# Nexenta/edge-fuse

Measured on NVIDIA H100. Metric: GiB/s hash+LZ4+dedup on 64 KiB chunks, higher is better.
Workload: dtype u8

## Files before the change

edge_fuse_b200/csrc/kernels.cu:

```cuda
#include "kernels.h"
#include "common.cuh"
#include "fingerprint.cuh"
#include "lz4_encode.cuh"
#include "lz4_encode_ring.cuh"
#include <type_traits>
#include "lz4_decode.cuh"
#include "lz4_decode_cta.cuh"
#include "streamgen.cuh"

namespace cmb {


__host__ __device__ __forceinline__ unsigned long long fnv_addr(unsigned long long u, unsigned long long l) {
	unsigned long long h = 14695981039346656037ULL;
#pragma unroll
	for (int i = 0; i < 8; i++) { h = (h ^ ((u >> (8 * i)) & 0xFF)) * 0x100000001b3ULL; }
#pragma unroll
	for (int i = 0; i < 8; i++) { h = (h ^ ((l >> (8 * i)) & 0xFF)) * 0x100000001b3ULL; }
	return h;
}

__device__ __forceinline__ uint64_t home_slot(unsigned long long key, uint64_t cap) {
	unsigned long long z = key;
	z = (z ^ (z >> 32)) * 0xD6E8FEB86659FD93ULL;
// ... 282 lines not shown
constexpr float COST_FULL = 160.0f;
#ifdef CMB_ENC_TIMELINE
__device__ unsigned long long *g_enc_timeline;
__device__ __forceinline__ unsigned long long enc_clock() {
	unsigned long long t;
	asm volatile("mov.u64 %0, %%globaltimer;" : "=l"(t));
	return t;
}
#endif
__global__ void __launch_bounds__(COST_WARPS * 32, 4) k_cost(EncodeJob job) {
	__shared__ __align__(16) uint32_t smp[COST_WARPS][256 + 4];
	__shared__ uint16_t tab[COST_WARPS][COST_TAB];
	const int lane = threadIdx.x & 31, warp = threadIdx.x >> 5;
	uint32_t *s = smp[warp];
	uint16_t *h = tab[warp];
	const uint8_t *sb = reinterpret_cast<const uint8_t *>(s);
	const uint32_t o0 = ((uint32_t)lane & 3u) * 32u;
	const uint32_t win_stride = (job.nbytes / 8u) & ~15u;
	for (uint32_t i = blockIdx.x * COST_WARPS + warp; i < job.n; i += gridDim.x * COST_WARPS) {
		const uint4 *src = reinterpret_cast<const uint4 *>(job.pages + (size_t)i * job.page_stride + (lane >> 2) * win_stride + o0);
		const uint4 a = __ldg(src), c = __ldg(src + 1);
		bool live = true;
		if (job.slot_idx) {
			const uint32_t idx = job.slot_idx[i];
			live = idx != 0xffffffffu && job.table.slots[idx].seq == job.seq0 + job.seq_stride * i;
		}
		uint32_t bucket = 0;
		[[maybe_unused]] uint32_t est = 0;
		if (live) {
			const uint32_t w[9] = {a.x, a.y, a.z, a.w, c.x, c.y, c.z, c.w, __shfl_down_sync(CMB_FULL, a.x, 1)};
			__syncwarp();
			reinterpret_cast<uint4 *>(s)[2 * lane] = a;
			reinterpret_cast<uint4 *>(s)[2 * lane + 1] = c;
#pragma unroll
			for (uint32_t k = 0; k < 32; k++) {
				if (o0 + k >= COST_POS) break;
				const uint32_t g = __funnelshift_r(w[k >> 2], w[(k >> 2) + 1], (k & 3u) * 8u);
				h[(g * 2654435761u) >> 21] = (uint16_t)((uint32_t)lane * 32u + k);
			}
			__syncwarp();
			uint32_t starts = 0, lits = 0;
#pragma unroll
			for (uint32_t k = 0; k < 32; k++) {
				if (o0 + k >= COST_POS) break;
				const uint32_t p = (uint32_t)lane * 32u + k;
				const uint32_t g = __funnelshift_r(w[k >> 2], w[(k >> 2) + 1], (k & 3u) * 8u);
				const uint32_t q = h[(g * 2654435761u) >> 21] & 1023u;
				const bool m = q != p && (q & 127u) < COST_POS && __funnelshift_r(s[q >> 2], s[(q >> 2) + 1], (q & 3u) * 8u) == g;
				const bool cont = m && o0 + k > 0u && (q & 127u) > 0u && sb[p - 1] == sb[q - 1];
				starts += m && !cont;
				lits += !m;
			}
#pragma unroll
			for (int d = 16; d > 0; d >>= 1) {
				starts += __shfl_xor_sync(CMB_FULL, starts, d);
				lits += __shfl_xor_sync(CMB_FULL, lits, d);
			}
			const float cost = (float)starts + COST_LIT * (float)lits / (float)job.accel;
			bucket = min(ENC_BUCKETS - 1u, (uint32_t)(cost * ((float)ENC_BUCKETS / COST_FULL)));
			est = starts << 16 | lits;
		}
		if (lane == 0) {
			const uint32_t pos = atomicAdd(&job.work[1 + bucket], 1u);
			job.order[(size_t)bucket * job.n + pos] = i;
#ifdef CMB_ENC_TIMELINE
			if (g_enc_timeline) g_enc_timeline[4 * (size_t)i + 3] = (unsigned long long)bucket << 32 | est;
#endif
		}
	}
}

__device__ __noinline__ uint32_t enc_ticket_chunk(const unsigned int *work, const uint32_t *order, uint32_t n, uint32_t t, int lane) {
	uint32_t cum = lane < (int)ENC_BUCKETS ? work[ENC_BUCKETS - lane] : 0u;
#pragma unroll
	for (int d = 1; d < (int)ENC_BUCKETS; d <<= 1) {
		const uint32_t v = __shfl_up_sync(CMB_FULL, cum, d);
		if (lane >= d) cum += v;
	}
	const int k = __ffs(__ballot_sync(CMB_FULL, lane < (int)ENC_BUCKETS && t < cum)) - 1;
	const uint32_t before = __shfl_sync(CMB_FULL, cum, (k + 31) & 31);
	return order[(size_t)(ENC_BUCKETS - 1 - k) * n + (t - (k ? before : 0u))];
}

constexpr int ENC_PLAIN_WARPS = 7, ENC_PLAIN_CTAS = 2, ENC_RING_WARPS = 13;
template <bool WIDE, int ENC>
__global__ void __launch_bounds__(ENC == 1 ? ENC_RING_WARPS * 32 : ENC_PLAIN_WARPS * 32, ENC == 1 ? 1 : ENC_PLAIN_CTAS) k_encode(EncodeJob job) {
	extern __shared__ __align__(128) uint8_t smem[];
	const int lane = threadIdx.x & 31, warp = threadIdx.x >> 5;
	const uint32_t nwarps = blockDim.x >> 5;
	uint8_t *wsm = smem + (size_t)warp * LZ4_TABLE_BYTES;
	PageRing ring;
	if (ENC == 1)
		ring_setup(ring, smem + (size_t)nwarps * LZ4_TABLE_BYTES + (size_t)warp * RING_ALLOC,
		    smem + (size_t)nwarps * (LZ4_TABLE_BYTES + RING_ALLOC) + (size_t)warp * RING_MBAR_BYTES, lane);
	const uint32_t gw = blockIdx.x * (blockDim.x >> 5) + warp;
	const bool direct = job.slot_idx != nullptr && job.arena.seg_bytes != 0u && job.accel != 0u && gw < ARENA_SEG_SLOTS;
	const uint32_t worst = (uint32_t)((24u + job.stage_stride + 15u) & ~15ull);
	unsigned long long seg_cur = 0, seg_end = 0;
	if (direct && lane == 0) { seg_cur = job.arena.seg[2 * gw]; seg_end = job.arena.seg[2 * gw + 1]; }
#ifdef CMB_ENC_TIMELINE
	uint32_t prev = ~0u;
#endif
	for (;;) {
		uint32_t i = 0;
		if (lane == 0) i = atomicAdd(job.work, 1u);
		i = __shfl_sync(CMB_FULL, i, 0);
		if (i < job.n && job.order) i = enc_ticket_chunk(job.work, job.order, job.n, i, lane);
#ifdef CMB_ENC_TIMELINE
		if (lane == 0 && g_enc_timeline) {
			const unsigned long long t = enc_clock();
			if (prev != ~0u) g_enc_timeline[4 * (size_t)prev + 2] = t;
			if (i < job.n) { g_enc_timeline[4 * (size_t)i] = gw; g_enc_timeline[4 * (size_t)i + 1] = t; }
			prev = i;
		}
#endif
		if (i >= job.n) break;
		const bool store = job.slot_idx != nullptr;
		uint32_t idx = 0;
		if (store) {
			idx = job.slot_idx[i];
			bool live = idx != 0xffffffffu && job.table.slots[idx].seq == job.seq0 + job.seq_stride * i;
			if (!live) { if (lane == 0) job.lens[i] = -1; continue; }
		}
		const uint8_t *src = job.pages + (size_t)i * job.page_stride;
		uint64_t fp_hi = 0, fp_lo = 0;
		if (job.accel == 0) {
			if (job.fps) {
				warp_fingerprint128(src, job.nbytes, lane, fp_hi, fp_lo);
				if (lane == 0) { job.fps[2 * (size_t)i] = fp_hi; job.fps[2 * (size_t)i + 1] = fp_lo; }
			}
			if (lane == 0) job.lens[i] = 0;
			if (store) commit_record(job, i, idx, src, job.nbytes, 0, true, fp_hi, fp_lo, lane);
			continue;
		}
		uint8_t *dst = job.stage + (size_t)(store ? gw : i) * job.stage_stride;
		unsigned long long base = 0;
		int in_arena = 0;
		if (direct) {
			if (lane == 0) {
				if (seg_cur + worst > seg_end) {
					if (seg_end > seg_cur) atomicAdd(job.arena.garbage, seg_end - seg_cur);
					const unsigned long long off = atomicAdd(job.arena.head, (unsigned long long)job.arena.seg_bytes);
					if (off + job.arena.seg_bytes <= job.arena.size) { seg_cur = off; seg_end = off + job.arena.seg_bytes; }
					else { seg_cur = seg_end = 0; }
				}
				in_arena = seg_cur + worst <= seg_end;
				base = seg_cur;
			}
			in_arena = __shfl_sync(CMB_FULL, in_arena, 0);
			base = __shfl_sync(CMB_FULL, base, 0);
			if (in_arena) dst = job.arena.base + base + 24;
		}
		uint32_t clen, ck = 0xffffffffu;
		if (job.fps) {
			clen = lz4_encode_lean<WIDE, true, ENC == 1>(src, job.nbytes, dst, job.accel, wsm, ring, lane, fp_hi, fp_lo, ck);
			if (lane == 0) { job.fps[2 * (size_t)i] = fp_hi; job.fps[2 * (size_t)i + 1] = fp_lo; }
		} else {
			clen = lz4_encode_lean<WIDE, false, ENC == 1>(src, job.nbytes, dst, job.accel, wsm, ring, lane, fp_hi, fp_lo, ck);
		}
		if (lane == 0) job.lens[i] = (int32_t)clen;
		if (store) {
			__syncwarp();
			if (in_arena) {
				const uint32_t used = commit_direct(job, i, idx, base, clen, fp_hi, fp_lo, lane);
				if (lane == 0) seg_cur += used;
				ckpt_store(job, idx, base, clen, ck, lane);
			} else {
				const unsigned long long at = commit_record(job, i, idx, dst, clen, (int32_t)clen, false, fp_hi, fp_lo, lane);
				if (at != ~0ull) ckpt_store(job, idx, at, clen, ck, lane);
			}
		}
	}
	if (direct && lane == 0) { job.arena.seg[2 * gw] = seg_cur; job.arena.seg[2 * gw + 1] = seg_end; }
}

static int g_sm_count = 0;
int sm_count() {
	if (!g_sm_count) {
		int dev = 0;
		cudaGetDevice(&dev);
		cudaDeviceGetAttribute(&g_sm_count, cudaDevAttrMultiProcessorCount, dev);
		if (g_sm_count <= 0) g_sm_count = 132;
	}
	return g_sm_count;
}

static int launch_encode_kernel(const EncodeJob &job, bool ring, cudaStream_t st) {
	const bool wide = job.nbytes >= LZ4_NARROW_LIMIT;
	void (*const kern)(EncodeJob) = ring ? (wide ? k_encode<true, 1> : k_encode<false, 1>)
	                                     : (wide ? k_encode<true, 0> : k_encode<false, 0>);
	const int warps = ring ? ENC_RING_WARPS : ENC_PLAIN_WARPS, ctas_per_sm = ring ? 1 : ENC_PLAIN_CTAS;
	const size_t smem = (size_t)warps * (ring ? RING_WARP_SMEM : LZ4_TABLE_BYTES);
	CMB_CHECK(cudaFuncSetAttribute(kern, cudaFuncAttributeMaxDynamicSharedMemorySize, (int)smem));
	uint32_t grid = (uint32_t)(sm_count() * ctas_per_sm);
	uint32_t need = (job.n + warps - 1) / warps;
	if (grid > need) grid = need;
	kern<<<grid, warps * 32, smem, st>>>(job);
	CMB_CHECK(cudaGetLastError());
	return 0;
}

int launch_encode(const EncodeJob &job_in, cudaStream_t st) {
	if (job_in.n == 0) return 0;
	EncodeJob job = job_in;
	const bool ring = job.accel >= 1 && job.accel <= RING_MAX_ACCEL && job.nbytes < (1u << 24);
	const uint32_t resident = (uint32_t)sm_count() * (ring ? ENC_RING_WARPS : ENC_PLAIN_CTAS * ENC_PLAIN_WARPS);
	if (job.n <= resident || job.accel == 0 || job.nbytes < 1024u) job.order = nullptr;
	CMB_CHECK(cudaMemsetAsync(job.work, 0, (job.order ? 1 + ENC_BUCKETS : 1) * sizeof(unsigned int), st));
	if (job.order) {
		k_cost<<<(job.n + COST_WARPS - 1) / COST_WARPS, COST_WARPS * 32, 0, st>>>(job);
		CMB_CHECK(cudaGetLastError());
	}
	if (launch_encode_kernel(job, ring, st) != 0) return -1;
	return job.order ? 2 : 1;
}

#ifdef CMB_ENC_TIMELINE
extern "C" int cmb200_enc_timeline(void *buf) {
	return cudaMemcpyToSymbol(g_enc_timeline, &buf, sizeof(buf)) == cudaSuccess ? 0 : -1;
}
#endif


__global__ void __launch_bounds__(256, 8) k_decode(DecodeJob job) {
	const int lane = threadIdx.x & 31;
	const uint32_t i = blockIdx.x * (blockDim.x >> 5) + (threadIdx.x >> 5);
	if (i >= job.n) return;
	uint8_t *out = job.pages + (size_t)i * job.nbytes;
	if (job.rec_off) {
		if (job.status[i] != ST_HIT) return;
		const unsigned long long off = job.rec_off[i];
		const uint8_t *rec = (off & REC_HOST) ? job.host + (off & ~REC_HOST) : job.arena + off;
		if ((off & REC_HOST) && lane == 0) {
			atomicAdd(job.host_hits, 1ull);
			hot_log(job.hot, job.addr[2 * (size_t)i], job.addr[2 * (size_t)i + 1]);
		}
		uint32_t clen = job.vlen[i] - 1u;
		if (clen == 0) {
			warp_copy_ro(out, rec + 24, job.nbytes, lane);
			return;
		}
		int used = lz4_decode_warp(rec + 24, clen, out, job.nbytes, lane);
		if (used != (int)clen && lane == 0) job.status[i] = ST_BAD_DECODE;
	} else {
		int used = lz4_decode_warp(job.blocks + (size_t)i * job.block_stride, (uint32_t)job.lens[i], out,
		    job.nbytes, lane);
		if (lane == 0) job.status[i] = used;
	}
}

int launch_decode(const DecodeJob &job, cudaStream_t st) {
	if (job.n == 0) return 0;
	const int warps = 8;
	k_decode<<<(job.n + warps - 1) / warps, warps * 32, 0, st>>>(job);
	CMB_CHECK(cudaGetLastError());
	return 0;
}


constexpr uint32_t GS_THREADS = DC_THREADS;
constexpr uint32_t GS_CTRL = 128 + 1152;
static_assert(sizeof(DecodeCta) <= 1152, "decoder state fits its slot");
constexpr uint32_t GS_MAX_PAGE = 65536;
constexpr uint32_t GS_PAIR_MAX_PAGE = 131072;
struct GetShared {
	unsigned long long bar;
	unsigned long long off;
	int32_t st;
	uint32_t clen;
	uint32_t owner;
	uint32_t idx;
	uint32_t region;
	uint32_t sections;
	uint32_t ck[CKPT_WORDS];
};
static_assert(sizeof(GetShared) <= 128, "control block");
__host__ __device__ inline uint32_t gs_recbuf(uint32_t nbytes) { return (24u + nbytes + 1024u + 31u) & ~15u; }
bool get_small_supports(uint32_t nbytes) { return nbytes >= 64u && nbytes <= GS_PAIR_MAX_PAGE && (nbytes & 15u) == 0; }
size_t get_small_smem(uint32_t nbytes) {
	return nbytes > GS_MAX_PAGE ? GS_CTRL + gs_recbuf(nbytes) : GS_CTRL + gs_recbuf(nbytes) + nbytes;
}
uint32_t get_small_region_entries(uint32_t nbytes) { return dc_region(nbytes); }

__device__ __forceinline__ unsigned long long ldv64(const unsigned long long *p) { return *reinterpret_cast<const volatile unsigned long long *>(p); }
__device__ __forceinline__ uint32_t ldv32(const uint32_t *p) { return *reinterpret_cast<const volatile uint32_t *>(p); }

__device__ void gs_lookup(const GetJob &job, unsigned long long u, unsigned long long l, GetShared *sh) {
	int32_t st = ST_MISS;
	uint32_t clen = 0, owner = 0;
	unsigned long long off = 0;
	const uint32_t idx = table_find(job.table, fnv_addr(u, l));
	if (idx != 0xffffffffu) {
		const Slot *s = &job.table.slots[idx];
		const uint32_t vlen = ldv32(&s->vlen);
		const unsigned long long au = ldv64(&s->addr_u), al = ldv64(&s->addr_l);
		if (vlen != 0u) {
			if (au == u && al == l) { st = ST_HIT; __threadfence(); off = ldv64(&s->rec_off); clen = vlen - 1u; }
			else st = ST_BAD_ENTRY;
		} else {
			const unsigned long long ow = ldv64(&s->owner);
			if (ow != 0ull && au == u && al == l) {
				st = ST_REMOTE; owner = (uint32_t)ow;
				__threadfence();
				off = ldv64(&s->rec_off);
				const uint32_t len1 = ldv32(&s->alloc);
				clen = len1 ? len1 - 1u : 0xffffffffu;
			}
		}
	}
	sh->st = st; sh->clen = clen; sh->off = off; sh->owner = owner; sh->idx = idx;
}

__device__ uint32_t gs_region_take(const GetJob &job) {
	uint32_t smid;
	asm volatile("mov.u32 %0, %%smid;" : "=r"(smid));
	const uint32_t words = (job.pool_n + 31u) / 32u;
	for (uint32_t probe = 0; probe < (1u << 22); probe++) {
		const uint32_t w = (smid + probe) % words;
		const uint32_t live = w + 1u == words && (job.pool_n & 31u) ? (1u << (job.pool_n & 31u)) - 1u : 0xffffffffu;
		const uint32_t vacant = ~ldv32(&job.pool_bits[w]) & live;
		if (!vacant) continue;
		const uint32_t b = (uint32_t)__ffs(vacant) - 1u;
		if (!((atomicOr(&job.pool_bits[w], 1u << b) >> b) & 1u)) return w * 32u + b;
	}
	return 0xffffffffu;
}
__device__ void gs_region_give(const GetJob &job, uint32_t r) { atomicAnd(&job.pool_bits[r / 32u], ~(1u << (r & 31u))); }

__device__ void gs_sections(const GetJob &job, GetShared *sh, DecodeCta *dc, uint32_t clen, bool local) {
	const uint32_t n = job.nbytes, S = n / DC_CHAINS;
	bool use = false;
	if (local && job.table.ckpt) {
		const uint32_t *ck = job.table.ckpt + (size_t)sh->idx * CKPT_WORDS;
		const uint32_t want = ckpt_tag(sh->off, clen);
		if (ldv32(ck) == want) {
			__threadfence();
			for (uint32_t k = 1; k < CKPT_WORDS; k++) sh->ck[k] = ldv32(ck + k);
			__threadfence();
			use = ldv32(ck) == want;
		}
	}
	for (uint32_t c = 0; c < DC_CHAINS; c++) { dc->ip0[c] = 0xffffffffu; dc->op0[c] = 0; dc->op_end[c] = 0; dc->cnt[c] = 0; dc->ip1[c] = 0; dc->op1[c] = 0; }
	dc->err = 0;
	dc->ip0[0] = 0; dc->op0[0] = 0;
	uint32_t prev = 0;
	if (use) {
		for (uint32_t k = 1; k < DC_CHAINS; k++) {
			const uint32_t v = sh->ck[k];
			if (v == 0xffffffffu) continue;
			const uint32_t ip = v >> CKPT_POS_BITS, op = k * S + (v & ((1u << CKPT_POS_BITS) - 1u));
			if (ip >= clen || op >= n || op >= (k + 1u) * S || ip <= dc->ip0[prev]) { use = false; break; }
			dc->ip0[k] = ip; dc->op0[k] = op;
			dc->op_end[prev] = op;
			prev = k;
		}
	}
	if (!use) {
		for (uint32_t c = 1; c < DC_CHAINS; c++) dc->ip0[c] = 0xffffffffu;
		prev = 0;
	}
	dc->op_end[prev] = n;
	sh->sections = use ? DC_CHAINS : 1u;
}

__device__ bool gs_sections_fit(const DecodeCta *dc, uint32_t clen, uint32_t n) {
	if (dc->err) return false;
	uint32_t prev = 0;
	for (uint32_t c = 1; c < DC_CHAINS; c++) {
		if (dc->ip0[c] == 0xffffffffu) continue;
		if (dc->ip1[prev] != dc->ip0[c] || dc->op1[prev] != dc->op0[c]) return false;
		prev = c;
	}
// ... 819 lines not shown
```

edge_fuse_b200/csrc/lz4_encode.cuh:

```cuda
#pragma once
#include "common.cuh"
#include "fingerprint.cuh"

namespace cmb {

constexpr uint32_t LZ4_MIN_MATCH = 4;
constexpr uint32_t LZ4_TAIL_LITERALS = 5;
constexpr uint32_t LZ4_MATCH_FIND_MARGIN = 12;
constexpr uint32_t LZ4_MIN_INPUT = 13;
constexpr uint32_t LZ4_NARROW_LIMIT = 65536 + 11;
constexpr uint32_t LZ4_FAR = 65535;
constexpr uint32_t LZ4_TABLE_BYTES = 16384;

__device__ __forceinline__ uint32_t lz4_hash4(uint32_t v) { return (v * 2654435761u) >> 19; }
__device__ __forceinline__ uint32_t lz4_hash5(uint64_t v) {
	return (uint32_t)(((v << 24) * 889523592379ULL) >> 52);
}

__device__ __forceinline__ uint32_t lz4_probe_off(uint32_t k, uint32_t accel) {
	if (k == 0) return 0;
	uint32_t m = k - 1, q = m >> 6, r = m & 63u;
	return 1u + accel * m + 32u * q * (q - 1u) + q * r;
}

template <bool WIDE> struct Lz4Table;
template <> struct Lz4Table<false> {
	uint16_t *t;
	__device__ __forceinline__ uint32_t get(uint32_t h) const { return t[h]; }
	__device__ __forceinline__ void put(uint32_t h, uint32_t pos) const { t[h] = (uint16_t)pos; }
};
template <> struct Lz4Table<true> {
	uint32_t *t;
	__device__ __forceinline__ uint32_t get(uint32_t h) const { return t[h]; }
	__device__ __forceinline__ void put(uint32_t h, uint32_t pos) const { t[h] = pos; }
};

struct Lz4Around { uint32_t before, at, next; };
struct Lz4Words { uint32_t w0, w1, w2, w3, sh; };
__device__ __forceinline__ Lz4Words lz4_around_load(const uint8_t *src, uint32_t p) {
	const uint32_t a = p & ~3u;
	const uint32_t *q = reinterpret_cast<const uint32_t *>(src + a);
	Lz4Words w;
	w.w0 = __ldg(q - (a != 0u));
	w.w1 = __ldg(q); w.w2 = __ldg(q + 1); w.w3 = __ldg(q + 2);
	w.sh = (p & 3u) * 8u;
	return w;
}
__device__ __forceinline__ Lz4Around lz4_around_align(const Lz4Words &w) {
	Lz4Around r;
	r.before = __funnelshift_r(w.w0, w.w1, w.sh);
	r.at = __funnelshift_r(w.w1, w.w2, w.sh);
	r.next = __funnelshift_r(w.w2, w.w3, w.sh);
	return r;
}
__device__ __forceinline__ Lz4Around lz4_around(const uint8_t *src, uint32_t p) {
	return lz4_around_align(lz4_around_load(src, p));
}


__device__ __noinline__ uint32_t lz4_emit_len(uint8_t *dst, uint32_t op, uint32_t count, int lane) {
	uint32_t nff = count / 255u;
	for (uint32_t i = lane; i < nff; i += 32) dst[op + i] = 0xFF;
	if (lane == 0) dst[op + nff] = (uint8_t)(count - nff * 255u);
	return op + nff + 1;
}
__device__ __forceinline__ uint32_t lz4_len_bytes(uint32_t count) { return count >= 15u ? (count - 15u) / 255u + 1u : 0u; }
__device__ __forceinline__ uint32_t lz4_seq_bytes(uint32_t lit, uint32_t mc) {
	return 3u + lit + lz4_len_bytes(lit) + lz4_len_bytes(mc);
}

__device__ __noinline__ void lz4_copy_literals(uint8_t *dst, const uint8_t *src, uint32_t len, int lane) {
	warp_copy_ro(dst, src, len, lane);
}

__device__ __noinline__ uint32_t lz4_count_long(const uint8_t *src, uint32_t a, uint32_t b, uint32_t lim,
    uint32_t lim4, int lane) {
	{
		const uint32_t pa = a + (uint32_t)lane;
		const bool same = pa < lim && ldg8(src + pa) == ldg8(src + b + (uint32_t)lane);
		const uint32_t stop = __ballot_sync(CMB_FULL, !same);
		if (stop) return (uint32_t)(__ffs(stop) - 1);
	}
	uint32_t total = 32;
	for (;;) {
		const uint32_t pa = a + total + 16u * lane;
		uint32_t nb = 0;
		if (pa < lim) {
			const uint32_t avail = min(16u, lim - pa);
			const uint32_t pb = b + total + 16u * lane;
#pragma unroll
			for (uint32_t j = 0; j < 4; j++) {
				if (nb == 4u * j && 4u * j < avail) {
					uint32_t x = read32u(src, pa + 4u * j, lim4) ^ read32u(src, pb + 4u * j, lim4);
					nb += x ? (uint32_t)(__ffs(x) - 1) >> 3 : 4u;
				}
			}
			nb = min(nb, avail);
		}
		const uint32_t stop = __ballot_sync(CMB_FULL, nb < 16u);
		if (stop) {
			int f = __ffs(stop) - 1;
			return total + 16u * f + __shfl_sync(CMB_FULL, nb, f);
		}
		total += 512u;
	}
}

__device__ __noinline__ uint32_t lz4_catchup_long(const uint8_t *src, uint32_t ip, uint32_t match,
    uint32_t anchor, int lane) {
	uint32_t total = 0;
	for (;;) {
		uint32_t k = total + lane + 1;
		bool ok = ip >= anchor + k && match >= k && ldg8(src + ip - k) == ldg8(src + match - k);
		uint32_t fail = __ballot_sync(CMB_FULL, !ok);
		if (fail) return total + (uint32_t)(__ffs(fail) - 1);
		total += 32;
	}
}

__device__ __forceinline__ uint64_t lz4_pack(bool found, bool retest, uint32_t ip, uint32_t match) {
	return ((uint64_t)found << 63) | ((uint64_t)retest << 62) | ((uint64_t)ip << 32) | match;
}

template <bool WIDE>
__device__ __noinline__ uint64_t lz4_search_slow(const uint8_t *src, uint32_t lim4, Lz4Table<WIDE> tab,
    uint32_t anchor, uint32_t shift, uint32_t accel, uint32_t mflimit, uint32_t g0, int lane, bool specials = true) {
	const uint32_t p0 = anchor + 1;
	for (;; g0 += 32) {
		const uint32_t g = g0 + lane;
		const bool special = g < shift;
		const uint32_t k = g - shift;
		uint32_t pos = p0 + lz4_probe_off(k, accel);
		const uint32_t nxt = p0 + lz4_probe_off(k + 1, accel);
		bool en = nxt <= mflimit;
		if (special) { pos = anchor - 2u + 2u * g; en = specials; }
		uint32_t h = 0x10000u + lane, pseq = 0, cand = 0;
		if (en) {
			if (WIDE) { uint64_t v = read64u(src, pos, lim4); pseq = (uint32_t)v; h = lz4_hash5(v); }
			else { pseq = read32u(src, pos, lim4); h = lz4_hash4(pseq); }
			cand = tab.get(h);
		}
		const uint32_t peers = __match_any_sync(CMB_FULL, h);
		const uint32_t lower = peers & ((1u << lane) - 1u);
		const uint32_t prev_pos = __shfl_sync(CMB_FULL, pos, lower ? 31 - __clz(lower) : lane);
		if (lower) cand = prev_pos;
		bool hit = false;
		if (en && !(special && g == 0) && cand + LZ4_FAR >= pos)
			hit = read32u(src, cand, lim4) == pseq;
		const uint32_t hits = __ballot_sync(CMB_FULL, hit);
		const uint32_t enmask = __ballot_sync(CMB_FULL, en);
		const int w = hits ? __ffs(hits) - 1 : 31;
		const uint32_t commit = hits ? (0xffffffffu >> (31 - w)) & enmask : enmask;
		if ((commit >> lane) & 1u) {
			const uint32_t pc = peers & commit;
			if (31 - __clz(pc) == lane) tab.put(h, pos);
		}
		__syncwarp();
		if (hits)
			return lz4_pack(true, g0 + (uint32_t)w < shift, __shfl_sync(CMB_FULL, pos, w),
			    __shfl_sync(CMB_FULL, cand, w));
		if (__ballot_sync(CMB_FULL, en || special) != CMB_FULL) return 0;
	}
}

__device__ __noinline__ uint32_t lz4_emit_general(uint8_t *dst, uint32_t op, const uint8_t *src, uint32_t anchor,
    uint32_t lit, uint32_t off, uint32_t mc, int lane) {
	if (lane == 0) dst[op] = (uint8_t)((min(lit, 15u) << 4) | min(mc, 15u));
	op++;
	if (lit >= 15u) op = lz4_emit_len(dst, op, lit - 15u, lane);
	if (lit <= 256u) {
		for (uint32_t i = lane; i < lit; i += 32) st_out8(dst + op + i, ldg8(src + anchor + i));
	} else {
		warp_copy_ro(dst + op, src + anchor, lit, lane);
	}
	op += lit;
	if (lane == 0) { dst[op] = (uint8_t)off; dst[op + 1] = (uint8_t)(off >> 8); }
	op += 2;
	if (mc >= 15u) op = lz4_emit_len(dst, op, mc - 15u, lane);
	return op;
}

__device__ __forceinline__ void st_out8_if(bool p, uint8_t *ptr, uint32_t v) {
	asm volatile("{\n\t.reg .pred q;\n\tsetp.ne.u32 q, %2, 0;\n\t@q st.global.u8 [%0], %1;\n\t}" ::"l"(
	                 __cvta_generic_to_global(ptr)), "r"(v), "r"((uint32_t)p)
	             : "memory");
}

__device__ __forceinline__ void lz4_emit_seq(uint8_t *dst, const uint8_t *src, uint32_t op, uint32_t from, uint32_t lit,
    uint32_t off, uint32_t mc, uint32_t b0, uint32_t b1, int lane) {
	if (lit <= 64u && mc < 15u + 255u) {
		uint8_t *o = dst + op;
		const uint32_t lext = lit >= 15u, mext = mc >= 15u;
		const uint32_t hl = 1u + lext;
		st_out8_if((uint32_t)lane < lit, o + hl + lane, b0);
		st_out8_if((uint32_t)lane + 32u < lit, o + hl + 32u + lane, b1);
		const uint32_t tail = hl + lit;
		const uint32_t head4 = (min(lit, 15u) << 4) | min(mc, 15u) | (((lit - 15u) & 0xffu) << 8) | (off << 16);
		const uint32_t val = lane < 4 ? head4 >> (8u * (uint32_t)lane) : mc - 15u;
		const uint32_t at = lane < 2 ? (uint32_t)lane : tail + (uint32_t)lane - 2u;
		const uint32_t owners = 0x0du | (lext << 1) | (mext << 4);
		st_out8_if((owners >> lane) & 1u, o + at, val);
	} else {
		lz4_emit_general(dst, op, src, from, lit, off, mc, lane);
	}
}


}
```

edge_fuse_b200/csrc/lz4_encode_ring.cuh:

```cuda
#pragma once
#include "lz4_encode.cuh"
#include "kernels.h"

namespace cmb {

constexpr uint32_t RING_BYTES = 1024, RING_BUF = 256, RING_BUFS = 4;
constexpr uint32_t RING_MIRROR = 16;
constexpr uint32_t RING_ALLOC = RING_BYTES + 64;
constexpr uint32_t RING_AHEAD = 376;
constexpr uint32_t RING_MAX_ACCEL = 12;
constexpr uint32_t RING_MBAR_BYTES = 64;
constexpr uint32_t RING_WARP_SMEM = LZ4_TABLE_BYTES + RING_ALLOC + RING_MBAR_BYTES;

__device__ __forceinline__ uint32_t smem_addr(const void *p) { return (uint32_t)__cvta_generic_to_shared(p); }
__device__ __forceinline__ void mbar_init(uint32_t bar, uint32_t arrivals) {
	asm volatile("mbarrier.init.shared::cta.b64 [%0], %1;" ::"r"(bar), "r"(arrivals) : "memory");
}
__device__ __forceinline__ void mbar_expect_tx(uint32_t bar, uint32_t bytes) {
	asm volatile("mbarrier.arrive.expect_tx.shared::cta.b64 _, [%0], %1;" ::"r"(bar), "r"(bytes) : "memory");
}
__device__ __forceinline__ void tma_load_1d(uint32_t dst, const void *src, uint32_t bytes, uint32_t bar) {
	asm volatile("cp.async.bulk.shared::cluster.global.mbarrier::complete_tx::bytes [%0], [%1], %2, [%3];" ::"r"(dst),
	    "l"(src), "r"(bytes), "r"(bar)
	    : "memory");
}
__device__ __forceinline__ bool mbar_try_wait(uint32_t bar, uint32_t parity) {
	uint32_t ok;
	asm volatile("{\n\t.reg .pred p;\n\tmbarrier.try_wait.parity.shared::cta.b64 p, [%1], %2;\n\tselp.u32 %0, 1, 0, p;\n\t}"
	    : "=r"(ok)
	    : "r"(bar), "r"(parity)
	    : "memory");
	return ok != 0;
}

struct PageRing {
	const uint8_t *bytes;
	uint32_t s_bytes;
	uint32_t s_bar;
	uint32_t issued;
	uint32_t ready;
	uint32_t parity;
};

__device__ __forceinline__ void ring_wait_buf(uint32_t s_bar, uint32_t &parity, uint32_t g) {
	const uint32_t r = g & (RING_BUFS - 1u);
	while (!mbar_try_wait(s_bar + 8u * r, (parity >> r) & 1u)) {}
	parity ^= 1u << r;
}

__device__ __forceinline__ void ring_setup(PageRing &ring, uint8_t *ring_smem, uint8_t *bar_smem, int lane) {
	ring.bytes = ring_smem;
	ring.s_bytes = smem_addr(ring_smem);
	ring.s_bar = smem_addr(bar_smem);
	ring.issued = ring.ready = 0;
	ring.parity = 0;
	if (lane == 0) {
#pragma unroll
		for (uint32_t r = 0; r < RING_BUFS; r++) mbar_init(ring.s_bar + 8u * r, 1u);
		asm volatile("fence.mbarrier_init.release.cluster;" ::: "memory");
		asm volatile("fence.proxy.async.shared::cta;" ::: "memory");
	}
	__syncwarp();
}

__device__ __noinline__ uint64_t ring_advance(uint32_t s_bytes, uint32_t s_bar, uint64_t state, const uint8_t *src,
    uint32_t n, uint32_t nbufs, uint32_t g_lo, int lane) {
	uint32_t issued = (uint32_t)state & 0xffffu, ready = (uint32_t)(state >> 16) & 0xffffu, parity = (uint32_t)(state >> 32);
	const uint32_t g_hi = min(g_lo + 2u, nbufs - 1u);
	const uint32_t upto = min(issued, g_hi + 1u);
	while (ready < upto) { ring_wait_buf(s_bar, parity, ready); ready++; }
	if (issued < g_lo) { issued = g_lo; ready = g_lo; }
	const uint32_t want = min(g_lo + RING_BUFS, nbufs);
	__syncwarp();
	if (lane == 0) {
		for (uint32_t g = issued; g < want; g++) {
			const uint32_t r = g & (RING_BUFS - 1u);
			const uint32_t nb = min(RING_BUF, (n - g * RING_BUF + 15u) & ~15u);
			const uint8_t *from = src + (size_t)g * RING_BUF;
			mbar_expect_tx(s_bar + 8u * r, nb + (r == 0u ? RING_MIRROR : 0u));
			tma_load_1d(s_bytes + r * RING_BUF, from, nb, s_bar + 8u * r);
			if (r == 0u) tma_load_1d(s_bytes + RING_BYTES, from, RING_MIRROR, s_bar);
		}
	}
	if (issued < want) issued = want;
	while (ready <= g_hi) { ring_wait_buf(s_bar, parity, ready); ready++; }
	return (uint64_t)issued | ((uint64_t)ready << 16) | ((uint64_t)parity << 32);
}
__device__ __forceinline__ void ring_step(PageRing &ring, const uint8_t *src, uint32_t n, uint32_t nbufs, uint32_t g_lo,
    int lane) {
	const uint64_t st = ring_advance(ring.s_bytes, ring.s_bar,
	    (uint64_t)ring.issued | ((uint64_t)ring.ready << 16) | ((uint64_t)ring.parity << 32), src, n, nbufs, g_lo, lane);
	ring.issued = (uint32_t)st & 0xffffu; ring.ready = (uint32_t)(st >> 16) & 0xffffu; ring.parity = (uint32_t)(st >> 32);
}
__device__ __forceinline__ void ring_drain(PageRing &ring) {
	while (ring.ready < ring.issued) { ring_wait_buf(ring.s_bar, ring.parity, ring.ready); ring.ready++; }
}

__device__ __forceinline__ Lz4Around ring_around(const uint8_t *ring, uint32_t p) {
	const uint32_t sh = (p & 3u) * 8u;
	const uint32_t *q = reinterpret_cast<const uint32_t *>(ring + (((p & ~3u) - 4u) & (RING_BYTES - 1u)));
	const uint32_t w0 = q[0], w1 = q[1], w2 = q[2], w3 = q[3];
	Lz4Around r;
	r.before = __funnelshift_r(w0, w1, sh);
	r.at = __funnelshift_r(w1, w2, sh);
	r.next = __funnelshift_r(w2, w3, sh);
	return r;
}

template <bool WIDE, bool FP, bool RING>
__device__ uint32_t lz4_encode_lean(const uint8_t *__restrict__ src, uint32_t n, uint8_t *__restrict__ dst,
    uint32_t accel, uint8_t *tab_smem, PageRing &ring, int lane, uint64_t &fp_hi, uint64_t &fp_lo, uint32_t &ck) {
	Lz4Table<WIDE> tab;
	tab.t = reinterpret_cast<decltype(tab.t)>(tab_smem);
	const uint32_t lim4 = (n + 3u) & ~3u;
	uint32_t op = 0, anchor = 0;
	const uint32_t ck_span = n / CKPT_WORDS;
	uint32_t ck_k = 1, ck_at = ck_span ? ck_span : 0xffffffffu;
	ck = 0xffffffffu;
	EfFrontier fp;
	if (FP) fp.start(src, n, lane);

	{
		uint4 z = make_uint4(0, 0, 0, 0);
		uint4 *t4 = reinterpret_cast<uint4 *>(tab_smem);
#pragma unroll 4
		for (uint32_t i = lane; i < LZ4_TABLE_BYTES / 16; i += 32) t4[i] = z;
	}
	__syncwarp();

	if (n >= LZ4_MIN_INPUT) {
		const uint32_t mflimit = n - LZ4_MATCH_FIND_MARGIN;
		const uint32_t mlimit = n - LZ4_TAIL_LITERALS;
		const uint32_t nbufs = (n + RING_BUF - 1u) / RING_BUF;
		const uint8_t *const rb = ring.bytes;
		if (RING) ring.issued = ring.ready = 0;
		const bool special = lane < 2;
		const uint32_t kk = (uint32_t)lane - 2u;
		uint32_t delta2 = special ? 2u * (uint32_t)lane - 2u : 1u + (kk ? 1u + accel * (kk - 1u) : 0u);
		const uint32_t need2 = 2u + accel * kk;
		uint32_t en_below = special ? 0u : (mflimit >= need2 ? mflimit - need2 + 1u : 0u);
		const uint32_t special_on = special ? 0xffffffffu : 0u;
		asm volatile("" : "+r"(delta2), "+r"(en_below));
		bool started = false;
		constexpr uint32_t NARROW_W = 16u;
		constexpr int NARROW_HIT = 12;
		uint32_t width = 32u, calm = 0u;
		uint32_t next_event = 0, ring_next = 0;
		uint32_t p_lit = 0, p_off = 0, p_mc = 0, litbyte = 0, litbyte2 = 0;
		for (;;) {
			if (anchor >= next_event) {
				while (anchor >= ck_at) {
					const uint32_t rel = anchor - ck_at;
					const uint32_t at = op + (started ? lz4_seq_bytes(p_lit, p_mc) : 0u);
					if ((uint32_t)lane == ck_k) ck = rel < ck_span ? (at << CKPT_POS_BITS) | rel : 0xffffffffu;
					ck_k++;
					ck_at = ck_k < CKPT_WORDS ? ck_at + ck_span : 0xffffffffu;
				}
				if (anchor >= ring_next) {
				if (RING) {
					const uint32_t g_lo = (max(anchor, 4u) - 4u) / RING_BUF;
					if (ring.ready == g_lo + 2u && ring.issued == g_lo + 3u && g_lo + 3u < nbufs) {
						__syncwarp();
						if (lane == 0) {
							const uint32_t g = g_lo + 3u, r = g & (RING_BUFS - 1u);
							const uint32_t nb = min(RING_BUF, (n - g * RING_BUF + 15u) & ~15u);
							const uint8_t *from = src + (size_t)g * RING_BUF;
							mbar_expect_tx(ring.s_bar + 8u * r, nb + (r == 0u ? RING_MIRROR : 0u));
							tma_load_1d(ring.s_bytes + r * RING_BUF, from, nb, ring.s_bar + 8u * r);
							if (r == 0u) tma_load_1d(ring.s_bytes + RING_BYTES, from, RING_MIRROR, ring.s_bar);
						}
						ring.issued = g_lo + 4u;
						ring_wait_buf(ring.s_bar, ring.parity, g_lo + 2u);
						ring.ready = g_lo + 3u;
					} else {
						ring_step(ring, src, n, nbufs, g_lo, lane);
					}
					ring_next = (g_lo + 1u) * RING_BUF + 4u;
				} else {
					ring_next = (anchor | 255u) + 1u;
				}
				if (FP) fp.upto(src, anchor + 512u, lane);
				}
				next_event = min(ring_next, ck_at);
			}
			const bool en = anchor < en_below && (uint32_t)lane < width;
			const uint32_t pos = en ? anchor + delta2 : 0u;
			const Lz4Around ai = RING ? ring_around(rb, pos) : lz4_around(src, pos);

			const uint32_t pseq = ai.at;
			const uint32_t h = WIDE ? lz4_hash5((uint64_t)ai.at | ((uint64_t)ai.next << 32)) : lz4_hash4(ai.at);
			const uint32_t cand = tab.get(h);
			__syncwarp();
			if (en) tab.put(h, pos);
			__syncwarp();
			Lz4Words acw = lz4_around_load(src, cand);
			const uint32_t seen = tab.get(h);
			__syncwarp();

			if (started) {
				lz4_emit_seq(dst, src, op, anchor - LZ4_MIN_MATCH - p_mc - p_lit, p_lit, p_off, p_mc, litbyte, litbyte2, lane);
				op += lz4_seq_bytes(p_lit, p_mc);
			}
			if (RING) {
				litbyte = rb[(anchor + (uint32_t)lane) & (RING_BYTES - 1u)];
				litbyte2 = rb[(anchor + 32u + (uint32_t)lane) & (RING_BYTES - 1u)];
			} else {
				litbyte = ldg8(src + min(anchor + (uint32_t)lane, n - 1u));
				litbyte2 = ldg8(src + min(anchor + 32u + (uint32_t)lane, n - 1u));
			}
			asm volatile("" : "+r"(acw.w0), "+r"(acw.w1), "+r"(acw.w2), "+r"(acw.w3));
			const Lz4Around ac = lz4_around_align(acw);
			const bool foreign = en && seen != (WIDE ? pos : (pos & 0xffffu));
			bool hit = en && lane != 0 && ac.at == pseq;
			if (WIDE) hit = hit && cand + LZ4_FAR >= pos;
			const uint32_t foreigns = __ballot_sync(CMB_FULL, foreign);
			const uint32_t hits = __ballot_sync(CMB_FULL, hit);
			uint32_t nf, nb;
			{
				const uint32_t xf = ai.next ^ ac.next;
				nf = xf ? (uint32_t)(__ffs(xf) - 1) >> 3 : 4u;
				nf = min(nf, mlimit - min(pos + LZ4_MIN_MATCH, mlimit));
				const uint32_t xb = ai.before ^ ac.before;
				nb = xb ? (uint32_t)__clz(xb) >> 3 : 4u;
				nb = min(nb, min(pos - min(anchor, pos), cand));
				if (special) nb = 0;
			}
			const uint32_t low_hit = hits & (0u - hits), low_for = foreigns & (0u - foreigns);
			uint32_t ip, match, fwd, back;
			bool retest_hit;
			if (low_hit - 1u < low_for - 1u) {
				const int w = __ffs(hits) - 1;
				const uint32_t pos_w = __shfl_sync(CMB_FULL, pos, w);
				if (en && lane > w && !(foreign && seen <= (WIDE ? pos_w : (pos_w & 0xffffu)))) tab.put(h, cand);
				__syncwarp();
				ip = pos_w;
				match = __shfl_sync(CMB_FULL, cand, w);
				fwd = __shfl_sync(CMB_FULL, nf, w);
				back = __shfl_sync(CMB_FULL, nb, w);
				retest_hit = w == 1;
				calm = w < NARROW_HIT ? calm + 1u : 0u;
				if (w >= NARROW_HIT) width = 32u; else if (calm >= 8u) width = NARROW_W;
				if (fwd == 4u || back == 4u) {
					if (fwd == 4u) fwd = 4u + lz4_count_long(src, ip + 8u, match + 8u, mlimit, lim4, lane);
					if (back == 4u && ip >= anchor + 5u && match >= 5u)
						back = 4u + lz4_catchup_long(src, ip - 4u, match - 4u, anchor, lane);
				}
			} else {
				uint64_t res = 0;
				const uint32_t enmask = __ballot_sync(CMB_FULL, en || special || (uint32_t)lane >= width);
				const uint32_t w0 = width;
				width = 32u; calm = 0u;
				if (foreigns) {
					if (en) tab.put(h, cand);
					__syncwarp();
					res = lz4_search_slow<WIDE>(src, lim4, tab, anchor, 2u, accel, mflimit, 0, lane, started);
				} else if (enmask == CMB_FULL) {
					res = lz4_search_slow<WIDE>(src, lim4, tab, anchor, 2u, accel, mflimit, w0, lane, started);
				}
				if (!(res >> 63)) break;
				retest_hit = (res >> 62) & 1u;
				ip = (uint32_t)(res >> 32) & 0x3fffffffu;
				match = (uint32_t)res;
				fwd = lz4_count_long(src, ip + LZ4_MIN_MATCH, match + LZ4_MIN_MATCH, mlimit, lim4, lane);
				back = retest_hit ? 0u : lz4_catchup_long(src, ip, match, anchor, lane);
			}
			p_off = ip - match;
			p_mc = back + fwd;
			p_lit = ip - back - anchor;
			const uint32_t end = ip + LZ4_MIN_MATCH + fwd;

			anchor = end;
			started = true;
			en_below |= special_on;
			if (end > mflimit) break;
		}
		if (started && anchor > mflimit) {
			lz4_emit_seq(dst, src, op, anchor - LZ4_MIN_MATCH - p_mc - p_lit, p_lit, p_off, p_mc, litbyte, litbyte2, lane);
			op += lz4_seq_bytes(p_lit, p_mc);
		}
		if (RING) ring_drain(ring);
	}

	while (ck_k < CKPT_WORDS && ck_span) {
		const uint32_t rel = anchor - ck_at;
		if ((uint32_t)lane == ck_k) ck = (anchor >= ck_at && rel < ck_span) ? (op << CKPT_POS_BITS) | rel : 0xffffffffu;
		ck_k++;
		ck_at += ck_span;
	}

	uint32_t run = n - anchor;
	if (lane == 0) dst[op] = (uint8_t)(min(run, 15u) << 4);
	op++;
	if (run >= 15u) op = lz4_emit_len(dst, op, run - 15u, lane);
	lz4_copy_literals(dst + op, src + anchor, run, lane);
	op += run;
	if (FP) fp.finish(src, n, lane, fp_hi, fp_lo);
	return op;
}

}
```

Before: 131.5.

## Stage literals as per-lane words and use aligned word loads in match counting

Literal prefetch now loads one funnel-shifted 32-bit word per lane instead of two bytes, so a warp keeps up to 128 literal bytes in registers and the fast register emit path covers runs up to 128. The long match counter loads five aligned words per side and funnel-shifts them, replacing per-step unaligned read32u calls and dropping the avail guard. It also adds optional clock64 phase profiling behind CMB_ENC_PHASES. This trades more loads and registers per step for fewer byte loads and fewer fallbacks to the general literal copy.

```diff
diff --git a/edge_fuse_b200/csrc/kernels.cu b/edge_fuse_b200/csrc/kernels.cu
--- a/edge_fuse_b200/csrc/kernels.cu
+++ b/edge_fuse_b200/csrc/kernels.cu
@@ -458,6 +458,10 @@
 			if (in_arena) dst = job.arena.base + base + 24;
 		}
 		uint32_t clen, ck = 0xffffffffu;
+#ifdef CMB_ENC_PHASES
+		if (lane == 0) s_enc_phase_row[warp] = g_enc_phases && gw % 4u == 0u ? g_enc_phases + 2u * ENC_PH_N * (size_t)i : nullptr;
+		__syncwarp();
+#endif
 		if (job.fps) {
 			clen = lz4_encode_lean<WIDE, true, ENC == 1>(src, job.nbytes, dst, job.accel, wsm, ring, lane, fp_hi, fp_lo, ck);
 			if (lane == 0) { job.fps[2 * (size_t)i] = fp_hi; job.fps[2 * (size_t)i + 1] = fp_lo; }
@@ -524,6 +528,12 @@
 #ifdef CMB_ENC_TIMELINE
 extern "C" int cmb200_enc_timeline(void *buf) {
 	return cudaMemcpyToSymbol(g_enc_timeline, &buf, sizeof(buf)) == cudaSuccess ? 0 : -1;
+}
+#endif
+#ifdef CMB_ENC_PHASES
+extern "C" int cmb200_enc_phases(void *buf, uint32_t *nphases) {
+	if (nphases) *nphases = ENC_PH_N;
+	return cudaMemcpyToSymbol(g_enc_phases, &buf, sizeof(buf)) == cudaSuccess ? 0 : -1;
 }
 #endif
 
diff --git a/edge_fuse_b200/csrc/lz4_encode.cuh b/edge_fuse_b200/csrc/lz4_encode.cuh
--- a/edge_fuse_b200/csrc/lz4_encode.cuh
+++ b/edge_fuse_b200/csrc/lz4_encode.cuh
@@ -88,10 +88,18 @@
 		if (pa < lim) {
 			const uint32_t avail = min(16u, lim - pa);
 			const uint32_t pb = b + total + 16u * lane;
+			uint32_t wa[5], wb[5];
+			const uint32_t qa = pa & ~3u, qb = pb & ~3u;
+#pragma unroll
+			for (uint32_t k = 0; k < 5; k++) {
+				wa[k] = qa + 4u * k < lim4 ? ldg32(src + qa + 4u * k) : 0u;
+				wb[k] = qb + 4u * k < lim4 ? ldg32(src + qb + 4u * k) : 0u;
+			}
 #pragma unroll
 			for (uint32_t j = 0; j < 4; j++) {
-				if (nb == 4u * j && 4u * j < avail) {
-					uint32_t x = read32u(src, pa + 4u * j, lim4) ^ read32u(src, pb + 4u * j, lim4);
+				if (nb == 4u * j) {
+					const uint32_t x = __funnelshift_r(wa[j], wa[j + 1], (pa & 3u) * 8u) ^
+					    __funnelshift_r(wb[j], wb[j + 1], (pb & 3u) * 8u);
 					nb += x ? (uint32_t)(__ffs(x) - 1) >> 3 : 4u;
 				}
 			}
@@ -186,14 +194,16 @@
 	             : "memory");
 }
 
+constexpr uint32_t LZ4_LIT_REG = 128;
 __device__ __forceinline__ void lz4_emit_seq(uint8_t *dst, const uint8_t *src, uint32_t op, uint32_t from, uint32_t lit,
-    uint32_t off, uint32_t mc, uint32_t b0, uint32_t b1, int lane) {
-	if (lit <= 64u && mc < 15u + 255u) {
+    uint32_t off, uint32_t mc, uint32_t lw, int lane) {
+	if (lit <= LZ4_LIT_REG && mc < 15u + 255u) {
 		uint8_t *o = dst + op;
 		const uint32_t lext = lit >= 15u, mext = mc >= 15u;
 		const uint32_t hl = 1u + lext;
-		st_out8_if((uint32_t)lane < lit, o + hl + lane, b0);
-		st_out8_if((uint32_t)lane + 32u < lit, o + hl + 32u + lane, b1);
+		const uint32_t l4 = 4u * (uint32_t)lane;
+#pragma unroll
+		for (uint32_t k = 0; k < 4; k++) st_out8_if(l4 + k < lit, o + hl + l4 + k, lw >> (8u * k));
 		const uint32_t tail = hl + lit;
 		const uint32_t head4 = (min(lit, 15u) << 4) | min(mc, 15u) | (((lit - 15u) & 0xffu) << 8) | (off << 16);
 		const uint32_t val = lane < 4 ? head4 >> (8u * (uint32_t)lane) : mc - 15u;
diff --git a/edge_fuse_b200/csrc/lz4_encode_ring.cuh b/edge_fuse_b200/csrc/lz4_encode_ring.cuh
--- a/edge_fuse_b200/csrc/lz4_encode_ring.cuh
+++ b/edge_fuse_b200/csrc/lz4_encode_ring.cuh
@@ -107,6 +107,40 @@
 	return r;
 }
 
+#ifdef CMB_ENC_PHASES
+enum : uint32_t {
+	ENC_PH_HEAD,
+	ENC_PH_EVENTS,
+	ENC_PH_TABLE,
+	ENC_PH_EMIT,
+	ENC_PH_WAIT,
+	ENC_PH_RESOLVE,
+	ENC_PH_SEARCH_SLOW,
+	ENC_PH_COUNT_LONG,
+	ENC_PH_CATCHUP_LONG,
+	ENC_PH_EMIT_GENERAL,
+	ENC_PH_N
+};
+__device__ unsigned long long *g_enc_phases;
+__shared__ unsigned long long *s_enc_phase_row[32];
+struct EncPhaseClock {
+	unsigned long long *row;
+	unsigned long long t;
+	__device__ __forceinline__ void start(int lane) {
+		row = lane == 0 ? s_enc_phase_row[threadIdx.x >> 5] : nullptr;
+		t = clock64();
+	}
+	__device__ __forceinline__ void mark(uint32_t ph) {
+		const unsigned long long now = clock64();
+		if (row) { atomicAdd(row + ph, now - t); atomicAdd(row + ENC_PH_N + ph, 1ull); }
+		t = now;
+	}
+};
+#define ENC_PHASE(ph) phc.mark(ph)
+#else
+#define ENC_PHASE(ph) do {} while (0)
+#endif
+
 template <bool WIDE, bool FP, bool RING>
 __device__ uint32_t lz4_encode_lean(const uint8_t *__restrict__ src, uint32_t n, uint8_t *__restrict__ dst,
     uint32_t accel, uint8_t *tab_smem, PageRing &ring, int lane, uint64_t &fp_hi, uint64_t &fp_lo, uint32_t &ck) {
@@ -146,9 +180,14 @@
 		constexpr int NARROW_HIT = 12;
 		uint32_t width = 32u, calm = 0u;
 		uint32_t next_event = 0, ring_next = 0;
-		uint32_t p_lit = 0, p_off = 0, p_mc = 0, litbyte = 0, litbyte2 = 0;
+		uint32_t p_lit = 0, p_off = 0, p_mc = 0, litw = 0;
+#ifdef CMB_ENC_PHASES
+		EncPhaseClock phc;
+		phc.start(lane);
+#endif
 		for (;;) {
 			if (anchor >= next_event) {
+				ENC_PHASE(ENC_PH_HEAD);
 				while (anchor >= ck_at) {
 					const uint32_t rel = anchor - ck_at;
 					const uint32_t at = op + (started ? lz4_seq_bytes(p_lit, p_mc) : 0u);
@@ -182,7 +221,9 @@
 				if (FP) fp.upto(src, anchor + 512u, lane);
 				}
 				next_event = min(ring_next, ck_at);
-			}
+				ENC_PHASE(ENC_PH_EVENTS);
+			}
+			ENC_PHASE(ENC_PH_HEAD);
 			const bool en = anchor < en_below && (uint32_t)lane < width;
 			const uint32_t pos = en ? anchor + delta2 : 0u;
 			const Lz4Around ai = RING ? ring_around(rb, pos) : lz4_around(src, pos);
@@ -196,17 +237,22 @@
 			Lz4Words acw = lz4_around_load(src, cand);
 			const uint32_t seen = tab.get(h);
 			__syncwarp();
+			ENC_PHASE(ENC_PH_TABLE);
 
 			if (started) {
-				lz4_emit_seq(dst, src, op, anchor - LZ4_MIN_MATCH - p_mc - p_lit, p_lit, p_off, p_mc, litbyte, litbyte2, lane);
+				lz4_emit_seq(dst, src, op, anchor - LZ4_MIN_MATCH - p_mc - p_lit, p_lit, p_off, p_mc, litw, lane);
 				op += lz4_seq_bytes(p_lit, p_mc);
-			}
-			if (RING) {
-				litbyte = rb[(anchor + (uint32_t)lane) & (RING_BYTES - 1u)];
-				litbyte2 = rb[(anchor + 32u + (uint32_t)lane) & (RING_BYTES - 1u)];
-			} else {
-				litbyte = ldg8(src + min(anchor + (uint32_t)lane, n - 1u));
-				litbyte2 = ldg8(src + min(anchor + 32u + (uint32_t)lane, n - 1u));
+				ENC_PHASE(p_lit <= LZ4_LIT_REG && p_mc < 15u + 255u ? ENC_PH_EMIT : ENC_PH_EMIT_GENERAL);
+			}
+			{
+				const uint32_t sh = (anchor & 3u) * 8u;
+				if (RING) {
+					const uint32_t *q = reinterpret_cast<const uint32_t *>(rb + (((anchor & ~3u) + 4u * (uint32_t)lane) & (RING_BYTES - 1u)));
+					litw = __funnelshift_r(q[0], q[1], sh);
+				} else {
+					const uint32_t a = min((anchor & ~3u) + 4u * (uint32_t)lane, (n - 1u) & ~3u);
+					litw = __funnelshift_r(ldg32(src + a), ldg32(src + a + 4u), sh);
+				}
 			}
 			asm volatile("" : "+r"(acw.w0), "+r"(acw.w1), "+r"(acw.w2), "+r"(acw.w3));
 			const Lz4Around ac = lz4_around_align(acw);
@@ -229,6 +275,7 @@
 			uint32_t ip, match, fwd, back;
 			bool retest_hit;
 			if (low_hit - 1u < low_for - 1u) {
+				ENC_PHASE(ENC_PH_WAIT);
 				const int w = __ffs(hits) - 1;
 				const uint32_t pos_w = __shfl_sync(CMB_FULL, pos, w);
 				if (en && lane > w && !(foreign && seen <= (WIDE ? pos_w : (pos_w & 0xffffu)))) tab.put(h, cand);
@@ -241,11 +288,18 @@
 				calm = w < NARROW_HIT ? calm + 1u : 0u;
 				if (w >= NARROW_HIT) width = 32u; else if (calm >= 8u) width = NARROW_W;
 				if (fwd == 4u || back == 4u) {
-					if (fwd == 4u) fwd = 4u + lz4_count_long(src, ip + 8u, match + 8u, mlimit, lim4, lane);
-					if (back == 4u && ip >= anchor + 5u && match >= 5u)
+					ENC_PHASE(ENC_PH_RESOLVE);
+					if (fwd == 4u) {
+						fwd = 4u + lz4_count_long(src, ip + 8u, match + 8u, mlimit, lim4, lane);
+						ENC_PHASE(ENC_PH_COUNT_LONG);
+					}
+					if (back == 4u && ip >= anchor + 5u && match >= 5u) {
 						back = 4u + lz4_catchup_long(src, ip - 4u, match - 4u, anchor, lane);
+						ENC_PHASE(ENC_PH_CATCHUP_LONG);
+					}
 				}
 			} else {
+				ENC_PHASE(ENC_PH_WAIT);
 				uint64_t res = 0;
 				const uint32_t enmask = __ballot_sync(CMB_FULL, en || special || (uint32_t)lane >= width);
 				const uint32_t w0 = width;
@@ -257,12 +311,15 @@
 				} else if (enmask == CMB_FULL) {
 					res = lz4_search_slow<WIDE>(src, lim4, tab, anchor, 2u, accel, mflimit, w0, lane, started);
 				}
+				ENC_PHASE(ENC_PH_SEARCH_SLOW);
 				if (!(res >> 63)) break;
 				retest_hit = (res >> 62) & 1u;
 				ip = (uint32_t)(res >> 32) & 0x3fffffffu;
 				match = (uint32_t)res;
 				fwd = lz4_count_long(src, ip + LZ4_MIN_MATCH, match + LZ4_MIN_MATCH, mlimit, lim4, lane);
+				ENC_PHASE(ENC_PH_COUNT_LONG);
 				back = retest_hit ? 0u : lz4_catchup_long(src, ip, match, anchor, lane);
+				ENC_PHASE(ENC_PH_CATCHUP_LONG);
 			}
 			p_off = ip - match;
 			p_mc = back + fwd;
@@ -272,10 +329,11 @@
 			anchor = end;
 			started = true;
 			en_below |= special_on;
+			ENC_PHASE(ENC_PH_RESOLVE);
 			if (end > mflimit) break;
 		}
 		if (started && anchor > mflimit) {
-			lz4_emit_seq(dst, src, op, anchor - LZ4_MIN_MATCH - p_mc - p_lit, p_lit, p_off, p_mc, litbyte, litbyte2, lane);
+			lz4_emit_seq(dst, src, op, anchor - LZ4_MIN_MATCH - p_mc - p_lit, p_lit, p_off, p_mc, litw, lane);
 			op += lz4_seq_bytes(p_lit, p_mc);
 		}
 		if (RING) ring_drain(ring);
```

Result: faster. 140.4 (median of 6 runs) (+6.8%).
